# se-hwan/landing-controller

Hardware: AMD Instinct MI355X
Metric: landing NLPs solved/sec (SRBM, N=40, batch) (higher is better)
Workload: dtype f64

## Files before the change

landing-controller_amd/csrc/ipm_core.hpp:

```cpp
#pragma once
#include <hip/hip_runtime.h>
#include <math.h>

#include "../../include/landing_nlp.h"

namespace landing {

enum { RSUM = 0, RMAX = 1, RMIN = 2 };
__device__ __forceinline__ double red_op(double a, double b, int op) { return op == RSUM ? a + b : (op == RMAX ? fmax(a, b) : fmin(a, b)); }
template <int K>
__device__ __forceinline__ void block_reduce(double (&v)[K], const int (&op)[K], double* red) {
  const int tid = threadIdx.x, nwave = (blockDim.x + 63) >> 6;
  for (int i = 0; i < K; ++i) {
#pragma unroll
    for (int mask = 32; mask >= 1; mask >>= 1) v[i] = red_op(v[i], __shfl_xor(v[i], mask), op[i]);
  }
  if ((tid & 63) == 0) for (int i = 0; i < K; ++i) red[(tid >> 6) * K + i] = v[i];
  __syncthreads();
  for (int i = 0; i < K; ++i) {
    double r = red[i];
    for (int w = 1; w < nwave; ++w) r = red_op(r, red[w * K + i], op[i]);
    v[i] = r;
  }
  __syncthreads();
}
__device__ __forceinline__ double block_reduce1(double v, int op, double* red) {
  double a[1] = {v}; const int o[1] = {op};
  block_reduce<1>(a, o, red);
  return a[0];
}

__device__ __forceinline__ void top4_push(double (&t)[4], double v) {
#pragma unroll
  for (int i = 0; i < 4; ++i) { const double hi = fmax(t[i], v); v = fmin(t[i], v); t[i] = hi; }
}
__device__ __forceinline__ void block_top4(double (&t)[4], double* red) {
  const int tid = threadIdx.x, nwave = (blockDim.x + 63) >> 6;
#pragma unroll
  for (int mask = 32; mask >= 1; mask >>= 1) {
    double o[4];
#pragma unroll
    for (int i = 0; i < 4; ++i) o[i] = __shfl_xor(t[i], mask);
#pragma unroll
    for (int i = 0; i < 4; ++i) top4_push(t, o[i]);
  }
  if ((tid & 63) == 0) for (int i = 0; i < 4; ++i) red[(tid >> 6) * 4 + i] = t[i];
  __syncthreads();
  for (int i = 0; i < 4; ++i) t[i] = red[i];
  for (int w = 1; w < nwave; ++w) for (int i = 0; i < 4; ++i) top4_push(t, red[w * 4 + i]);
  __syncthreads();
}

typedef double f64x4 __attribute__((vector_size(32)));

#if defined(__HIP_DEVICE_COMPILE__)
typedef const double __attribute__((address_space(1)))* landing_gptr;
#else
typedef const double* landing_gptr;
#endif

struct ElStep { double dz, dw, dn, da; };
__device__ __forceinline__ ElStep el_step(double sd, double a, double n, double z, double w, double mu, double rho_pen, double ds) {
  ElStep e;
  const double D = a + z * n / w, rn = z + w - rho_pen;
  e.dz = (mu - a * z - z * (mu - n * w + n * rn) / w - sd * z * ds) / D;
  e.dw = -e.dz - rn;
  e.dn = (mu - n * w - n * e.dw) / w;
  e.da = sd * ds + e.dn;
  return e;
}

struct IpmCtl {
  double mu, delta_last, th_max, c_pr, c_co, c_cm, c_ys, c_zs, c_nz, e_pr, e_du, e_co;
  double tau, omt, a_pr, a_du, th0, ph0, dphi, alpha, s_corr, delta, ft;
  long long tp;
  int nfilt, it, status, need_reg_streak, nreset, last_reset_it, ncrawl, clip_k_cur, last_mu_it, cutstreak, wd_count, first_failed, force_step;
  int accepted, armijo_step, fact_ok, skipped_zero, attempt;
  int stag, full_prev;
  double e_prev;
  int flag, fresh, ls_done, need_corr, fallback;
  int feas, feas_used, lim;
  int fjam, fstat; double v1_ref;
  double c_rn, f_vmax, f_v1;
  int n_feas, stalled, polished, hard_lim, want_entry; double th_entry, f_theq;
  double fdc;
};
enum { ACT_GO = 0, ACT_STOP = 1, ACT_RESET = 2, ACT_FEAS = 3, ACT_BACK = 4 };

__host__ __device__ __forceinline__ void ipm_init(IpmCtl& K, const landing_solver_opts& o) {
  K = IpmCtl{};
  K.mu = o.mu_init; K.c_nz = 1.0; K.omt = -1.0; K.e_prev = 1e300;
  K.status = LANDING_MAX_ITER; K.clip_k_cur = o.clip_k; K.lim = o.max_iter; K.hard_lim = o.max_iter > 0 ? 3 * o.max_iter : 0;
  K.fdc = o.feas_delta_dec > 0.0 ? o.feas_delta_dec : o.delta_dec;
}

__host__ __device__ __forceinline__ void ipm_errors(IpmCtl& K, const landing_solver_opts& o, double du) {
  const double pr = K.c_pr, co = K.c_co;
  if (K.feas) du = fmax(du, K.c_rn);
  K.e_pr = pr; K.e_du = du; K.e_co = co;
  if (o.stag_relief > 0) {
    const double E = fmax(pr, du);
    K.stag = (!K.feas && K.mu <= o.tol / 10.0 * 1.0000001 && K.full_prev && E > 0.5 * K.e_prev) ? K.stag + 1 : 0;
    K.e_prev = E;
  }
}

__host__ __device__ __forceinline__ void ipm_enter_phase(IpmCtl& K, const landing_solver_opts& o) {
  const int it = K.it;
  K.feas = 1; K.n_feas++; K.feas_used = K.n_feas >= o.feas_max ? 1 : 0; K.status = LANDING_MAX_ITER; K.lim = it + o.max_iter; if (K.lim > K.hard_lim) K.lim = K.hard_lim; K.fstat = -1; K.fjam = 0; K.want_entry = 1; K.fdc = o.feas_delta_dec > 0.0 ? o.feas_delta_dec : o.delta_dec;
  K.mu = o.mu_init; K.nfilt = 0; K.th_max = 0.0; K.delta_last = 0.0; K.need_reg_streak = 0; K.cutstreak = 0; K.force_step = 0; K.wd_count = 0;
  K.it = it + 1;
}

__host__ __device__ __forceinline__ void ipm_leave_phase(IpmCtl& K, const landing_solver_opts& o) {
  const int it = K.it;
  K.feas = 0; K.lim = it + (o.max_iter > 1 ? o.max_iter : 1); if (K.lim > K.hard_lim) K.lim = K.hard_lim; K.status = LANDING_MAX_ITER;
  K.mu = (o.feas_ret_push > 0.0 && o.feas_ret_mu > 0.0) ? o.feas_ret_mu : o.mu_init; K.fjam = 0; K.nfilt = 0; K.delta_last = 0.0; K.need_reg_streak = 0; K.wd_count = 0; K.th_max = 0.0; K.nreset = 0; K.last_reset_it = it; K.ncrawl = 0;
  K.cutstreak = 0; K.force_step = 0;
  K.it = it + 1;
}

__host__ __device__ __forceinline__ void ipm_restart(IpmCtl& K, const landing_solver_opts& o, bool stalled, bool lost) {
  const int it = K.it, nreset = K.nreset;
  K.last_reset_it = it;
  if (stalled) K.ncrawl++;
  K.nreset = nreset + 1;
  K.fresh = (((o.fresh_restart & 2) && nreset + 1 == 2) || ((o.fresh_restart & 1) && nreset + 1 == 1 && !stalled && !lost)) ? 1 : 0;
  if (K.fresh) { if (K.clip_k_cur > 1) K.clip_k_cur = 2; K.th_max = 0.0; }
  K.mu = o.mu_init; K.nfilt = 0; K.delta_last = 0.0; K.need_reg_streak = 0; K.wd_count = 0;
  K.it = it + 1;
}

__host__ __device__ __forceinline__ int ipm_decide(IpmCtl& K, const landing_solver_opts& o, bool failed) {
  const double pr = K.e_pr, du = K.e_du, co = K.e_co, mu = K.mu;
  const int it = K.it, nreset = K.nreset;
  int act = ACT_GO;
  bool give_up = false;
  if (K.feas) {
    const bool conv = fmax(du, fmax(pr, co)) <= o.tol;
    if (!(du < 1e300) || !(pr < 1e300) || !(co < 1e300)) { K.status = LANDING_NUMERICAL; act = ACT_STOP; }
    else if (K.f_vmax <= 1e-9 && pr <= o.tol) act = ACT_BACK;
    else if (conv && K.f_v1 > o.feas_cert) { K.status = LANDING_INFEASIBLE; act = ACT_STOP; }
    else if (conv) act = ACT_BACK;
    else if (o.feas_back > 0.0 && !K.feas_used && K.f_v1 + K.f_theq <= o.feas_back * K.th_entry) act = ACT_BACK;
    else if (o.feas_stat > 0) {
      const double v1 = K.f_v1;
      if (K.fstat < 0 || !(fabs(v1 - K.v1_ref) <= 0.05 * K.v1_ref)) { K.v1_ref = v1; K.fstat = 0; } else K.fstat++;
      if (K.fstat >= o.feas_stat && mu <= 1e-4 && pr <= 1e-3) {
        if (v1 <= o.feas_cert) act = ACT_BACK;
        else if (o.feas_polish > 0.0 && !K.polished) {
          K.polished = 1; K.fstat = -1; K.delta_last = o.feas_polish / (o.feas_delta_dec > 0.0 ? o.feas_delta_dec : o.delta_dec); K.need_reg_streak = 2;
        }
        else if (o.feas_resume && !K.stalled) { K.stalled = 1; K.feas_used = 1; act = ACT_BACK; }
        else { K.status = LANDING_STALLED; act = ACT_STOP; }
      }
    }
    if (act == ACT_GO && it >= K.lim) act = ACT_STOP;
    if (act == ACT_BACK) ipm_leave_phase(K, o);
  }
  else if (failed) { K.status = LANDING_NUMERICAL; give_up = true; }
  else if (!(du < 1e300) || !(pr < 1e300) || !(co < 1e300)) { K.status = LANDING_NUMERICAL; give_up = true; }
  else if (fmax(du, fmax(pr, co)) <= o.tol) { K.status = LANDING_CONVERGED; act = ACT_STOP; }
  else if (it >= K.lim) give_up = true;
  else if (du > o.reset_du && nreset >= o.max_resets && o.max_resets > 0) { K.status = LANDING_NUMERICAL; give_up = true; }
  else if (o.feas_jam > 0 && K.fjam >= o.feas_jam && pr > 1e-3 && o.feas_phase) { give_up = true; if (K.feas_used) K.stalled = 1; }
  else {
    const bool jam = du > o.reset_du && nreset < o.max_resets;
    const bool stalled = o.restart_period > 0 && it - K.last_reset_it >= o.restart_period && mu >= o.mu_init && nreset < o.max_resets && K.ncrawl < ((o.fresh_restart & 4) ? 2 : 1);
    const bool overreg = o.reset_delta > 0.0 && K.delta_last > o.reset_delta && nreset < o.max_resets;
    const bool lost = (o.fresh_restart & 8) && o.restart_period > 0 && mu < o.mu_init && pr > 1e-3 && nreset < o.max_resets &&
                      ((it - K.last_mu_it >= 2 * o.restart_period && it - K.last_reset_it >= o.restart_period) || K.wd_count >= 3);
    if (jam || stalled || overreg || lost) { act = ACT_RESET; ipm_restart(K, o, stalled, lost); }
  }
  if (give_up) {
    if (K.stalled) K.status = LANDING_STALLED;
    if (o.feas_phase && !K.feas_used && o.max_iter > 0 && it < K.hard_lim) {
      act = ACT_FEAS;
      ipm_enter_phase(K, o);
    } else act = ACT_STOP;
  }
  return act;
}

__host__ __device__ __forceinline__ bool ipm_barrier_update(IpmCtl& K, const landing_solver_opts& o, int nfree) {
  double sd = 1.0, sc = 1.0;
  if (o.barrier_smax > 0.0) {
    sd = fmax(o.barrier_smax, (K.c_ys + K.c_zs) / ((double)nfree + K.c_nz)) / o.barrier_smax;
    sc = fmax(o.barrier_smax, K.c_zs / K.c_nz) / o.barrier_smax;
  }
  const double mu = K.mu;
  if (fmax(K.e_du / sd, fmax(K.c_pr, K.c_cm / sc)) <= o.kappa_eps * mu && mu > o.tol / 10.0) {
    K.mu = fmax(o.tol / 10.0, fmin(o.kappa_mu * mu, pow(mu, o.theta_mu)));
    K.nfilt = 0; K.last_mu_it = K.it; K.wd_count = 0;
    return true;
  }
  K.tau = fmax(o.tau_min, 1.0 - mu);
  return false;
}

__host__ __device__ __forceinline__ double ipm_delta_dec(const IpmCtl& K, const landing_solver_opts& o) { return (K.feas && o.feas_delta_dec > 0.0) ? K.fdc : o.delta_dec; }

__host__ __device__ __forceinline__ void ipm_first_delta(IpmCtl& K, const landing_solver_opts& o, double dec, double floor) {
  const double dl = K.delta_last;
// ... 163 lines not shown
```

landing-controller_amd/csrc/solver_kernels.hip:

```cpp
#include <hip/hip_runtime.h>
#include <math.h>
#include <type_traits>

#include "../../include/landing_nlp.h"
#include "ipm_core.hpp"


namespace landing {

constexpr int NZ_JX = 0, NZ_JU = 157, NZ_JUN = 385, NZ_HX = 613, NZ_HU = 642, NZ_HUN = 802, NZ_TOT = 962;
constexpr int GS = 49;
constexpr int PS = 25;
constexpr int YS = 37;
constexpr int RIC_K = 0, RIC_KAP = 576, RIC_MT = 600, RIC_MV = 888, RIC_PX = 900, RIC_PV = 1188, RIC_STRIDE = 1200;
constexpr int RIC_FWD0 = 288, RIC_FWDN = 612;
constexpr int FILT_CAP = 64;
constexpr int SOLVER_NMAX = 96;
constexpr int SOLVER_THREADS = 256;
constexpr int RCG = 36;
constexpr int RUNC = 48;

constexpr int CX_SR = NZ_TOT + 48, CX_ONE = CX_SR + 208, CX_MONE = CX_ONE + 1, CX_ZERO = CX_ONE + 2, CX_LEN = CX_ONE + 3;
constexpr int ATAB_TB = 6, ATAB_LTMAX = 6;
constexpr int ASM_NSLOT = 512;
// ... 50 lines not shown

__device__ __forceinline__ MemberMem carve(const Layout& L, double* w) {
  MemberMem M;
  M.x = w; w += L.nx; M.xt = w; w += L.nx; M.dx = w; w += L.nx; M.gx = w; w += L.nx;
  M.g = w; w += L.ng; M.gt = w; w += L.ng; M.s = w; w += L.ng; M.ds = w; w += L.ng;
  M.zL = w; w += L.ng; M.zU = w; w += L.ng;
  M.y = w; w += L.ng; M.yn = w; w += L.ng;
  M.sig = w; w += L.ng; M.rho = w; w += L.ng;
  M.J = w; w += L.nnz_jac; M.H = w; w += L.nnz_hess; M.Hc = w; w += (size_t)L.N * RUNC; M.ric = w; w += (size_t)(L.N + 1) * RIC_STRIDE; M.cond = w; w += (size_t)L.N * RCG;
  M.en = w; w += L.ng; M.ep = w; w += L.ng; M.wn = w; w += L.ng; M.wp = w; w += L.ng;
  M.sig2 = w; w += L.ng; M.rho2 = w; w += L.ng;
  M.s2 = w; w += L.ng; M.zL2 = w; w += L.ng; M.zU2 = w; w += L.ng; M.y2 = w;
  return M;
}

__host__ __device__ __forceinline__ void mem_accept_swap(MemberMem& M) {
  double* t;
#define LANDING_SWAP(a, b) t = M.a; M.a = M.b; M.b = t
  LANDING_SWAP(s, s2); LANDING_SWAP(zL, zL2); LANDING_SWAP(zU, zU2); LANDING_SWAP(y, y2); LANDING_SWAP(sig, sig2); LANDING_SWAP(rho, rho2);
  LANDING_SWAP(g, gt); LANDING_SWAP(x, xt);
#undef LANDING_SWAP
}


constexpr int FWD_DXL_NMAX = 64;
constexpr int XCH = 112 * 4;
static_assert(2 * XCH >= 24 * YS, "A1 also holds Y (24 x YS)");
struct Lds {
  double G[48 * GS];
  double P[24 * PS];
  double A1[2 * XCH];
  double Ah[2 * 12 * YS];
  double gam[48], q[24], sig[24], w[48], dinv[24];
  double red[(SOLVER_THREADS / 64) * 9];
  double filt_th[FILT_CAP], filt_ph[FILT_CAP];
  double prof[32];
  int flag;
  int segb[SOLVER_NMAX * 8];
  double carry[ASM_NSLOT];
  double rcl[RCG];
  double jhl[CX_LEN];
  double dump[64];
  const unsigned long long* ctab; const unsigned long long* ccomb; int c_ml, c_mid, rc_on;
  double bnd_lb[36 + 2 * 104], bnd_ub[36 + 2 * 104];
  MemberMem M; Layout L; const double* p; int prof_on;
  IpmCtl ks;
  int clip_now, jamrun, action, fact_failed;
  int first_trial, fast;
  double nxt[6];
  unsigned long long atab_mid[ATAB_LTMAX * SOLVER_THREADS];
  unsigned long long acomb_mid[SOLVER_THREADS];
};
__shared__ Lds SH;
__device__ __forceinline__ MemberMem live_mem() {
  MemberMem M = SH.M;
#if defined(__HIP_DEVICE_COMPILE__)
  double** q = reinterpret_cast<double**>(&M);
#pragma unroll
  for (int i = 0; i < MEMBER_MEM_PTRS; ++i) {
    const unsigned long long a = (unsigned long long)q[i];
    const unsigned lo = (unsigned)__builtin_amdgcn_readfirstlane((int)(unsigned)a), hi = (unsigned)__builtin_amdgcn_readfirstlane((int)(unsigned)(a >> 32));
    q[i] = (double*)((unsigned long long)lo | ((unsigned long long)hi << 32));
  }
#endif
  return M;
}
static_assert(36 * FWD_DXL_NMAX + 12 <= 24 * PS + 2 * XCH + 2 * 12 * YS && offsetof(Lds, A1) == offsetof(Lds, P) + sizeof(double) * 24 * PS && offsetof(Lds, Ah) == offsetof(Lds, A1) + sizeof(double) * 2 * XCH,
              "dx (x layout, N <= FWD_DXL_NMAX) fits the adjacent arrays [P | A1 | A^] (forward_pass / row_products)");
static_assert(offsetof(Lds, atab_mid) <= 65528, "the assembly tables address G, A^, gamma, cx, the partial sums and the dump slots with 16-bit byte offsets");
__host__ __device__ inline unsigned long long aterm_pack(int pa, int pb, int pc, int d, bool keep, bool ah) {
  const unsigned lo = (unsigned)pa | ((unsigned)pb << 16);
  const unsigned hi = (unsigned)pc | (((unsigned)d | (keep ? 1u : 0u) | (ah ? 2u : 0u)) << 16);
  return (unsigned long long)lo | ((unsigned long long)hi << 32);
}
__host__ __device__ inline unsigned long long acomb_pack(int n, int s0, int d, bool ah) {
  return (unsigned long long)((unsigned)n | ((unsigned)s0 << 16)) | ((unsigned long long)((unsigned)d | (ah ? 2u : 0u)) << 32);
}

template <int KT, class FA, class FB>
__device__ __forceinline__ f64x4 mfma_tile(f64x4 c, FA fa, FB fb) {
  const int l = threadIdx.x & 63, ij = l & 15, kq = l >> 4;
#pragma unroll
  for (int kt = 0; kt < KT; ++kt) c = __builtin_amdgcn_mfma_f64_16x16x4f64(fa(ij, kt * 4 + kq), fb(kt * 4 + kq, ij), c, 0, 0, 0);
  return c;
}

__device__ __forceinline__ double fast_rcp(double d) {
  double i = __builtin_amdgcn_rcp(d);
  i = fma(i, fma(-d, i, 1.0), i);
  return fma(i, fma(-d, i, 1.0), i);
}

__device__ __forceinline__ double lane_bcast(double v, int src) {
  const int hi = __builtin_amdgcn_readlane(__double2hiint(v), src);
  const int lo = __builtin_amdgcn_readlane(__double2loint(v), src);
  return __hiloint2double(hi, lo);
}

template <int NU>
__device__ __noinline__ void gauss_jordan_wave(const double* G, const double* gam, double* Kl, double* kl, int* flag) {
  const int lane = threadIdx.x;
  double col[NU];
  const bool isUU = lane < NU, isUS = lane >= NU && lane < NU + 24, isG = lane == NU + 24;
  {
    const double* src = isG ? gam + 24 : G + 24 * GS + (isUU ? 24 + lane : (isUS ? lane - NU : 0));
    const int stride = isG ? 1 : GS;
#pragma unroll
    for (int i = 0; i < NU; ++i) col[i] = src[i * stride];
  }
  bool ok = true;
#pragma unroll 1
  for (int j = 0; j < NU; ++j) {
    const double d = lane_bcast(col[0], j);
    if (!(d > 0.0) || !(d < 1e300)) ok = false;
    double inv = __builtin_amdgcn_rcp(d);
    inv = fma(inv, fma(-d, inv, 1.0), inv);
    inv = fma(inv, fma(-d, inv, 1.0), inv);
    const double pj = col[0] * inv;
    double m[NU];
#pragma unroll
    for (int i = 1; i < NU; ++i) m[i] = lane_bcast(col[i], j);
    __builtin_amdgcn_sched_barrier(0);
#pragma unroll
    for (int i = 1; i < NU; ++i) col[i - 1] = fma(-m[i], pj, col[i]);
    col[NU - 1] = pj;
  }
  if (isUS) {
#pragma unroll
    for (int i = 0; i < NU; ++i) Kl[i * 24 + (lane - NU)] = col[i];
  }
  if (isG) {
#pragma unroll
    for (int i = 0; i < NU; ++i) kl[i] = col[i];
  }
  if (lane == 0) *flag = ok ? 1 : 0;
}

constexpr int ASM_SEG_LEN[7] = {NZ_JU - NZ_JX, NZ_JUN - NZ_JU, NZ_HX - NZ_JUN, NZ_HU - NZ_HX, NZ_HUN - NZ_HU, NZ_TOT - NZ_HUN, RUNC};
constexpr int ASM_SEG_POS[7] = {NZ_JX, NZ_JU, NZ_JUN, NZ_HX, NZ_HU, NZ_HUN, NZ_TOT};
static_assert(NZ_JUN - NZ_JU <= SOLVER_THREADS && 2 * 104 <= SOLVER_THREADS, "one load per thread and segment");
__device__ __forceinline__ int uni(int v) {
#if defined(__HIP_DEVICE_COMPILE__)
  return __builtin_amdgcn_readfirstlane(v);
#else
  return v;
#endif
}
template <class P>
__device__ __forceinline__ P uni_ptr(P q) {
  const unsigned long long a = (unsigned long long)q;
  return (P)((unsigned long long)(unsigned)uni((int)(unsigned)a) | ((unsigned long long)(unsigned)uni((int)(unsigned)(a >> 32)) << 32));
}
__device__ __forceinline__ double uni(double v) { return __hiloint2double(uni(__double2hiint(v)), uni(__double2loint(v))); }
struct SweepCtx {
  landing_gptr JH, SR, Gr, Cd;
  const unsigned long long* ctab; const unsigned long long* ccomb;
  int c_ml, c_mid, rc_on, ng;
};
__device__ __forceinline__ SweepCtx sweep_ctx() {
  const Lds& S = SH;
  SweepCtx X;
  X.JH = uni_ptr((landing_gptr)S.M.J); X.SR = uni_ptr((landing_gptr)S.M.sig); X.Gr = uni_ptr((landing_gptr)S.M.g); X.Cd = uni_ptr((landing_gptr)S.M.cond);
  X.ctab = uni_ptr(S.ctab); X.ccomb = uni_ptr(S.ccomb);
  X.c_ml = uni(S.c_ml); X.c_mid = uni(S.c_mid); X.rc_on = uni(S.rc_on); X.ng = uni(S.L.ng);
  return X;
}
struct AsmRegs { double jh[7], sr, g, rc; int tp; };
__device__ __forceinline__ void asm_issue(int k, const SweepCtx& X, AsmRegs& R) {
  const Lds& S = SH;
  const int tid = threadIdx.x, ng = X.ng;
  const int* sb = S.segb + k * 8;
  const int g0 = Layout::g_stage(k);
#pragma unroll
  for (int sgm = 0; sgm < 7; ++sgm) R.jh[sgm] = X.JH[uni(sb[sgm]) + (tid < ASM_SEG_LEN[sgm] ? tid : 0)];
  R.tp = uni(sb[7]);
  R.sr = X.SR[tid < 104 ? g0 + tid : (tid < 208 ? ng + g0 + tid - 104 : 0)];
  R.g = X.Gr[g0 + (tid < 12 ? tid : 0)];
  R.rc = 0.0;
  if (X.rc_on) R.rc = X.Cd[(size_t)k * RCG + (tid < RCG ? tid : 0)];
}
__device__ __forceinline__ void asm_copy(const AsmRegs& R) {
  Lds& S = SH;
  const int tid = threadIdx.x;
#pragma unroll
  for (int sgm = 0; sgm < 7; ++sgm) if (tid < ASM_SEG_LEN[sgm]) S.jhl[ASM_SEG_POS[sgm] + tid] = R.jh[sgm];
  if (tid < 208) S.jhl[CX_SR + tid] = R.sr;
}
__device__ __forceinline__ void asm_terms(const SweepCtx& X, int nb, const AsmRegs& R) {
  Lds& S = SH;
  const int tid = threadIdx.x, LT = X.c_ml, tp = R.tp;
  char* const lds0 = reinterpret_cast<char*>(&S);
  const unsigned ahoff = nb ? (unsigned)(12 * YS * sizeof(double)) : 0u;
  const bool mid = (tp == X.c_mid);
  const unsigned long long* gt = X.ctab + (size_t)tp * LT * SOLVER_THREADS;
  double acc = 0.0;
  for (int j0 = 0; j0 < LT; j0 += ATAB_TB) {
    unsigned long long t[ATAB_TB];
    if (mid) {
#pragma unroll
      for (int u = 0; u < ATAB_TB; ++u) t[u] = S.atab_mid[(j0 + u) * SOLVER_THREADS + tid];
    } else {
#pragma unroll
      for (int u = 0; u < ATAB_TB; ++u) t[u] = gt[(j0 + u) * SOLVER_THREADS + tid];
    }
    double a[ATAB_TB], b[ATAB_TB], c[ATAB_TB];
#pragma unroll
    for (int u = 0; u < ATAB_TB; ++u) {
      const unsigned lo = (unsigned)t[u], hi = (unsigned)(t[u] >> 32);
      a[u] = *reinterpret_cast<const double*>(lds0 + (lo & 0xffffu)); b[u] = *reinterpret_cast<const double*>(lds0 + (lo >> 16)); c[u] = *reinterpret_cast<const double*>(lds0 + (hi & 0xffffu));
    }
#pragma unroll
    for (int u = 0; u < ATAB_TB; ++u) {
      const unsigned dd = (unsigned)(t[u] >> 48);
      acc += a[u] * b[u] * c[u];
      *reinterpret_cast<double*>(lds0 + ((dd & 0xfff8u) + ((dd & 2u) ? ahoff : 0u))) = acc;
      acc = (dd & 1u) ? acc : 0.0;
    }
  }
  if (tid < 12) { const int i = tid; S.Ah[nb * (12 * YS) + (i < 6 ? i : (i < 9 ? i + 3 : i - 3)) * YS + (YS - 1)] = -R.g; }
  if (tid < RCG) S.rcl[tid] = R.rc;
}
__device__ __forceinline__ void asm_combine(const SweepCtx& X, int nb, const AsmRegs& R) {
  Lds& S = SH;
  const int tid = threadIdx.x, tp = R.tp;
  const unsigned long long code = tp == X.c_mid ? S.acomb_mid[tid] : X.ccomb[tp * SOLVER_THREADS + tid];
  const unsigned lo = (unsigned)code, dd = (unsigned)(code >> 32);
  const int n = (int)(lo & 7u);
  if (n > 0) {
    char* const lds0 = reinterpret_cast<char*>(&S);
    const double* sl = reinterpret_cast<const double*>(lds0 + (lo >> 16));
    double tot = 0.0;
    for (int i = 0; i < n; ++i) tot += sl[i];
    *reinterpret_cast<double*>(lds0 + ((dd & 0xfff8u) + ((dd & 2u) ? (nb ? (unsigned)(12 * YS * sizeof(double)) : 0u) : 0u))) = tot;
  }
}

#if defined(__HIP_DEVICE_COMPILE__)
typedef double __attribute__((address_space(1)))* landing_gptr_w;
#else
typedef double* landing_gptr_w;
#endif
__device__ __forceinline__ landing_gptr_w uniform_record(double* rec) { return uni_ptr((landing_gptr_w)rec); }

constexpr int G_GAMMA = GS - 1, P_PV = PS - 1, AH_B = YS - 1;
static_assert(G_GAMMA == 48 && P_PV == 24 && AH_B == 36, "spare columns of G / P / A^ hold gamma / p / b");

template <int NU>
struct StageLanes {
  int ct, lj, lk, c;
  bool isg, live, ym, pm, wr;
  bool am[3];
  int gb, cd384, cm;
  int yb, pa1, pb, p2, fb, ab[3];
  int xw, xw0, xcp, xcr;
  unsigned iK, iM, iP, rs;
  int sw, pw;
};
template <int NU>
__device__ __forceinline__ StageLanes<NU> stage_lanes() {
  constexpr int NR = NU + 24, D = (int)sizeof(double);
  constexpr int oG = (int)offsetof(Lds, G), oP = (int)offsetof(Lds, P), oAh = (int)offsetof(Lds, Ah), oA1 = (int)offsetof(Lds, A1);
  StageLanes<NU> Z;
  const int tid = threadIdx.x, l = tid & 63;
  Z.ct = uni(tid >> 6); Z.lj = l & 15; Z.lk = l >> 4;
  const int ct = Z.ct, lj = Z.lj, lk = Z.lk, c = 16 * ct + lj;
  Z.c = c;
  Z.isg = (c == NR); Z.live = (c <= NR);
  const bool isg = Z.isg, live = Z.live;
  const int cl = c < NR ? c : NR;
  const int cp = NU == 24 ? cl : (cl < NU ? cl : cl + (24 - NU));
  Z.ym = live && (c < 12 || c >= NU);
  int ycol = c < NU ? c + 24 : c - NU;
  ycol = Z.ym ? (isg ? AH_B : ycol) : 0;
  Z.pm = live && c >= 12 && (c < NU || isg);
  const int pcol = Z.pm ? (isg ? P_PV : c) : 0;
  Z.gb = oG + (cp + lk * GS) * D; Z.cd384 = (cp - lk) * ((GS - 1) * D); Z.cm = c - lk;
  Z.yb = oAh + (lk * YS + ycol) * D;
  Z.pa1 = oP + (lj * PS + lk) * D;
  Z.pb = oP + (lk * PS + pcol) * D;
#pragma unroll
  for (int rt = 0; rt < 3; ++rt) {
    const int rho = 16 * rt + lj;
    const int a = rho < NU ? 24 + rho : (rho < NR ? rho - NU : 36);
    Z.am[rt] = a < 36;
    Z.ab[rt] = oAh + (lk * YS + (Z.am[rt] ? a : 0)) * D;
  }
  Z.p2 = oP + ((12 + (lj < 12 ? lj : 11)) * PS + lk) * D;
  Z.fb = oAh + ((lj < 12 ? lj : 11) * YS + 24 + lk) * D;
  Z.xw = oA1 + (c * 4 + lk) * D; Z.xw0 = oA1 + (c * 4) * D; Z.xcp = oA1 + (64 * 4 + lk * 4 + lj) * D; Z.xcr = oA1 + (64 * 4 + lj * 4 + lk) * D;
  Z.wr = c >= NU && c <= NR;
  const unsigned sj = (unsigned)(c - NU), ulk = (unsigned)lk, rs = isg ? 1u : 24u;
  Z.rs = rs * D;
  Z.iK = ((isg ? (unsigned)RIC_KAP : (unsigned)RIC_K + sj) + ulk * rs) * D; Z.iM = ((isg ? (unsigned)RIC_MV : (unsigned)RIC_MT + sj) + ulk * rs) * D;
  Z.iP = ((isg ? (unsigned)RIC_PV : (unsigned)RIC_PX + sj) + ulk * rs) * D;
  const int scol = isg ? AH_B : (int)sj, pcw = isg ? P_PV : (int)sj;
  Z.sw = oAh + (lk * YS + scol) * D; Z.pw = oP + (lk * PS + pcw) * D;
  return Z;
}
__device__ __forceinline__ double lds_get(int boff) { return *reinterpret_cast<const double*>(reinterpret_cast<const char*>(&SH) + boff); }
__device__ __forceinline__ void lds_put(int boff, double v) { *reinterpret_cast<double*>(reinterpret_cast<char*>(&SH) + boff) = v; }

constexpr unsigned PIVOT_KEY_MAX = 0x7e37e43cu - 0x00100000u;
template <int STEP, int NU>
__device__ __forceinline__ unsigned pivot_block_step(f64x4 (&T)[3], const StageLanes<NU>& Z) {
  constexpr int OFF = 4 * STEP, D = (int)sizeof(double);
  static_assert((OFF >> 4) == ((OFF + 3) >> 4), "a pivot block lies inside one row tile");
  constexpr int RTB = OFF >> 4, R0 = (OFF & 15) >> 2;
  constexpr int WSZ = 64 * 4;
  static_assert(WSZ + 48 * 4 <= XCH, "exchange buffer");
  constexpr int XB = (STEP & 1) * XCH * D;
  constexpr int CB = (int)offsetof(Lds, A1) + XB + WSZ * D;
  const bool inblk = (unsigned)(Z.lj - (OFF & 15)) < 4u;
  lds_put(Z.xw + XB, T[RTB][R0]);
  if (Z.ct == RTB && inblk) {
#pragma unroll
    for (int rt = 0; rt < 3; ++rt)
#pragma unroll
      for (int r = 0; r < 4; ++r) lds_put(Z.xcp + XB + ((16 * rt + 4 * r) * 4 - (OFF & 15)) * D, T[rt][r]);
  }
  __syncthreads();
  double a[4][4];
#pragma unroll
  for (int i = 0; i < 4; ++i)
#pragma unroll
    for (int j = 0; j <= i; ++j) a[i][j] = lds_get(CB + ((OFF + i) * 4 + j) * D);
  double w[4];
#pragma unroll
  for (int i = 0; i < 4; ++i) w[i] = lds_get(Z.xw0 + XB + i * D);
  double am[3];
#pragma unroll
  for (int rt = 0; rt < 3; ++rt) { const double cv = lds_get(Z.xcr + XB + 16 * rt * 4 * D); am[rt] = (rt == RTB && inblk) ? 0.0 : cv; }
  auto recip = [](double d) { double i = __builtin_amdgcn_rcp(d); i = fma(i, fma(-d, i, 1.0), i); return fma(i, fma(-d, i, 1.0), i); };
  const double a00 = a[0][0], a10 = a[1][0], a11 = a[1][1], a20 = a[2][0], a21 = a[2][1], a22 = a[2][2], a30 = a[3][0], a31 = a[3][1], a32 = a[3][2], a33 = a[3][3];
  const double detA = fma(a00, a11, -a10 * a10), iA = recip(detA);
  const double e00 = fma(a20, a11, -a21 * a10) * iA, e01 = fma(a21, a00, -a20 * a10) * iA, e10 = fma(a30, a11, -a31 * a10) * iA, e11 = fma(a31, a00, -a30 * a10) * iA;
  const double s00 = fma(-e01, a21, fma(-e00, a20, a22)), s10 = fma(-e11, a21, fma(-e10, a20, a32)), s11 = fma(-e11, a31, fma(-e10, a30, a33));
  const double detS = fma(s00, s11, -s10 * s10), iS = recip(detS);
  unsigned hm = 0u;
  { const double piv[4] = {a00, detA, s00, detS};
#pragma unroll
    for (int j = 0; j < 4; ++j) { const unsigned h = (unsigned)__double2hiint(piv[j]) - 0x00100000u; hm = h > hm ? h : hm; } }
  const int lk = Z.lk;
  auto solve = [&](const double (&wv)[4]) {
    const double t2 = fma(-e01, wv[1], fma(-e00, wv[0], wv[2])), t3 = fma(-e11, wv[1], fma(-e10, wv[0], wv[3]));
    const double r2 = fma(s11, t2, -s10 * t3) * iS, r3 = fma(s00, t3, -s10 * t2) * iS;
    const double q0 = fma(a11, wv[0], -a10 * wv[1]) * iA, q1 = fma(a00, wv[1], -a10 * wv[0]) * iA;
    const double r0 = fma(-e10, r3, fma(-e00, r2, q0)), r1 = fma(-e11, r3, fma(-e01, r2, q1));
    return lk == 0 ? r0 : (lk == 1 ? r1 : (lk == 2 ? r2 : r3));
  };
  const double R = solve(w);
  if (16 * Z.ct + 16 > OFF) {
#pragma unroll
    for (int rt = 0; rt < 3; ++rt) T[rt] = __builtin_amdgcn_mfma_f64_16x16x4f64(am[rt], -R, T[rt], 0, 0, 0);
    T[RTB][R0] = R;
  }
  return hm;
}

__device__ __forceinline__ void rec_put(landing_gptr_w rec, unsigned boff, double v) {
#if defined(__HIP_DEVICE_COMPILE__)
  typedef char __attribute__((address_space(1)))* gchar_w;
  *reinterpret_cast<landing_gptr_w>(reinterpret_cast<gchar_w>(rec) + boff) = v;
#else
  *reinterpret_cast<double*>(reinterpret_cast<char*>(rec) + boff) = v;
#endif
}
template <int NU>
__device__ __forceinline__ bool stage_eliminate(const StageLanes<NU>& Z, const SweepCtx& X, landing_gptr_w rec, double delta, int k) {
  constexpr int NR = NU + 24, D = (int)sizeof(double);
  const int lk = Z.lk;
  const bool isg = Z.isg, live = Z.live, ym = Z.ym, pm = Z.pm;
  const int cb = k & 1;
  const int ah = cb * (12 * YS * D);
  f64x4 T[3];
  {
#pragma unroll
    for (int rt = 0; rt < 3; ++rt)
#pragma unroll
      for (int r = 0; r < 4; ++r) {
        const int rb = 16 * rt + 4 * r;
        if (rb < NR) {
          const int rp = NU == 24 ? rb : (rb < NU ? rb : rb + (24 - NU));
          const int m384 = rp * ((GS - 1) * D) < Z.cd384 ? rp * ((GS - 1) * D) : Z.cd384;
          const double v = lds_get(Z.gb + rp * D + m384) + (Z.cm == rb ? delta : 0.0);
          T[rt][r] = live ? v : 0.0;
        } else T[rt][r] = 0.0;
      }
    if (X.rc_on) {
      Lds& S = SH;
#pragma unroll
      for (int rt = 0; rt < 3; ++rt)
#pragma unroll
        for (int r = 0; r < 4; ++r) {
          const int rb = 16 * rt + 4 * r;
          if (rb < NR) {
            const int ab = rb < NU ? 24 + rb : rb - NU;
            static_assert(RCG % 4 == 0 && NU % 4 == 0, "a group of four rows lies on one side of every border");
            const double g = ab < RCG ? S.rcl[ab + lk] : 0.0;
            T[rt][r] += isg ? g : 0.0;
          }
        }
    }
  }
  {
    double be[3];
    {
      const int yb = Z.yb + ah;
#pragma unroll
      for (int kt = 0; kt < 3; ++kt) { const double v = lds_get(yb + 4 * kt * YS * D); be[kt] = ym ? v : 0.0; }
    }
    double pa1[3], add1[3];
#pragma unroll
    for (int kt = 0; kt < 3; ++kt) pa1[kt] = lds_get(Z.pa1 + 4 * kt * D);
#pragma unroll
    for (int r = 0; r < 3; ++r) { const double v = lds_get(Z.pb + 4 * r * PS * D); add1[r] = pm ? v : 0.0; }
    double av[3][3];
#pragma unroll
    for (int rt = 0; rt < 3; ++rt) {
      const int ab = Z.ab[rt] + ah;
#pragma unroll
      for (int kt = 0; kt < 3; ++kt) { const double v = lds_get(ab + 4 * kt * YS * D); av[rt][kt] = Z.am[rt] ? v : 0.0; }
    }
    double pa2[3], add2[3];
    if (NU == 24) {
#pragma unroll
      for (int kt = 0; kt < 3; ++kt) pa2[kt] = lds_get(Z.p2 + 4 * kt * D);
#pragma unroll
      for (int r = 0; r < 3; ++r) { const double v = lds_get(Z.pb + (12 + 4 * r) * PS * D); add2[r] = pm ? v : 0.0; }
    }
    f64x4 Y1 = {0.0, 0.0, 0.0, 0.0};
#pragma unroll
    for (int kt = 0; kt < 3; ++kt) Y1 = __builtin_amdgcn_mfma_f64_16x16x4f64(pa1[kt], be[kt], Y1, 0, 0, 0);
#pragma unroll
    for (int r = 0; r < 3; ++r) Y1[r] += add1[r];
#pragma unroll
    for (int rt = 0; rt < 3; ++rt)
#pragma unroll
      for (int kt = 0; kt < 3; ++kt) T[rt] = __builtin_amdgcn_mfma_f64_16x16x4f64(av[rt][kt], Y1[kt], T[rt], 0, 0, 0);
    if (NU == 24) {
      f64x4 Y2 = {0.0, 0.0, 0.0, 0.0};
#pragma unroll
      for (int kt = 0; kt < 3; ++kt) Y2 = __builtin_amdgcn_mfma_f64_16x16x4f64(pa2[kt], be[kt], Y2, 0, 0, 0);
#pragma unroll
      for (int r = 0; r < 3; ++r) Y2[r] += add2[r];
      T[0][3] += Y2[0]; T[1][0] += Y2[1]; T[1][1] += Y2[2];
    }
  }
  static_assert(NU == 12 || NU == 24, "3 or 6 block steps per stage");
  constexpr int SC = NU == 24 ? 3 : 1;
  AsmRegs nxt;
  const bool more = k > 0;
#define ASM_HOOK(step) do { if constexpr (SC == (step)) { if (more) asm_copy(nxt); } if constexpr (SC + 1 == (step)) { if (more) asm_terms(X, cb ^ 1, nxt); } if constexpr (SC + 2 == (step)) { if (more) asm_combine(X, cb ^ 1, nxt); } } while (0)
  unsigned key = pivot_block_step<0>(T, Z), kq;
#define KEY_MAX(e) do { kq = (e); key = kq > key ? kq : key; } while (0)
  if (more) asm_issue(k - 1, X, nxt);
  ASM_HOOK(1);
  KEY_MAX(pivot_block_step<1>(T, Z));
  ASM_HOOK(2);
  KEY_MAX(pivot_block_step<2>(T, Z));
  ASM_HOOK(3);
  if constexpr (NU == 24) {
    KEY_MAX(pivot_block_step<3>(T, Z));
    ASM_HOOK(4);
    KEY_MAX(pivot_block_step<4>(T, Z));
    ASM_HOOK(5);
    KEY_MAX(pivot_block_step<5>(T, Z));
  }
#undef KEY_MAX
#undef ASM_HOOK
  if (!((unsigned)uni((int)key) < PIVOT_KEY_MAX)) return false;
  f64x4 Mq = {0.0, 0.0, 0.0, 0.0};
  {
    const int fb = Z.fb + ah;
#pragma unroll
    for (int kt = 0; kt < 3; ++kt) Mq = __builtin_amdgcn_mfma_f64_16x16x4f64(lds_get(fb + 4 * kt * D), T[0][kt], Mq, 0, 0, 0);
  }
  if (Z.wr) {
    const int sw = Z.sw + ah;
#pragma unroll
    for (int r = 0; r < 3; ++r) rec_put(rec, Z.iM + (unsigned)(4 * r) * Z.rs, lds_get(sw + 4 * r * YS * D) - Mq[r]);
#pragma unroll
    for (int rt = 0; rt < 3; ++rt)
#pragma unroll
      for (int r = 0; r < 4; ++r) {
        const int rb = 16 * rt + 4 * r;
        const double v = T[rt][r];
        if (rb < NU) rec_put(rec, Z.iK + (unsigned)rb * Z.rs, v);
        else if (rb < NR) {
          lds_put(Z.pw + (rb - NU) * PS * D, v);
          if (rb - NU < 12) rec_put(rec, Z.iP + (unsigned)(rb - NU) * Z.rs, v);
        }
      }
  }
  return true;
}

__device__ __noinline__ bool last_stage_eliminate(double* rec_, double delta_, int k_) {
  const StageLanes<12> Z = stage_lanes<12>();
  const SweepCtx X = sweep_ctx();
  return stage_eliminate<12>(Z, X, uniform_record(rec_), uni(delta_), uni(k_));
}

template <bool TIMED>
__device__ __forceinline__ bool stage_loop(const StageLanes<24>& Z, const SweepCtx& X, landing_gptr_w rec, double delta, int k, int& n_try) {
  bool ok = true;
  for (; k >= 0 && ok; --k, rec -= RIC_STRIDE) {
    long long tb_ = 0;
    if (TIMED) tb_ = (long long)wall_clock64();
    ok = stage_eliminate<24>(Z, X, rec, delta, k);
    __syncthreads();
    ++n_try;
    if (TIMED) { const long long n_ = (long long)wall_clock64(); if (threadIdx.x == 0) SH.prof[PH_B_ELIM] += (double)(n_ - tb_); }
  }
  return ok;
}

__device__ __noinline__ bool riccati_backward(double delta) {
  Lds& S = SH;
  const Layout& L = S.L;
  const MemberMem& M = S.M;
  const double* p = S.p;
  const int N = L.N, lane = threadIdx.x, NT = blockDim.x;
  (void)p; (void)N; (void)lane; (void)NT;
  bool ok = true;
  int n_try = 0;
  for (int e = lane; e < 24 * PS; e += NT) S.P[e] = 0.0;
  __syncthreads();
  if (lane < 12) {
    const int i = lane;
    const int ra = i < 6 ? 12 + i : 24 + (i - 6), rb = i < 6 ? 18 + i : 30 + (i - 6);
    const double qn2 = S.ks.feas ? 0.0 : 2.0 * p[L.o_QN + i];
    S.P[i * PS + i] = qn2 + M.sig[ra] + M.sig[rb] + delta;
    S.P[i * PS + P_PV] = qn2 * (M.x[12 * N + i] - p[12 * N + i]) + M.rho[ra] + M.rho[rb];
    double* rec = M.ric + (size_t)N * RIC_STRIDE;
    for (int j = 0; j < 24; ++j) rec[RIC_PX + i * 24 + j] = (j == i) ? S.P[i * PS + i] : 0.0;
    rec[RIC_PV + i] = S.P[i * PS + P_PV];
  }
  for (int e = lane; e < 48 * GS; e += NT) S.G[e] = 0.0;
  for (int e = lane; e < 2 * 12 * YS; e += NT) S.Ah[e] = 0.0;
  __syncthreads();
  const SweepCtx X = sweep_ctx();
  const bool timed = uni(S.prof_on) != 0;
  {
    AsmRegs first;
    asm_issue(N - 1, X, first);
    asm_copy(first);
    __syncthreads();
    asm_terms(X, (N - 1) & 1, first);
    __syncthreads();
    asm_combine(X, (N - 1) & 1, first);
  }
  __syncthreads();
  {
    long long tb_ = timed ? (long long)wall_clock64() : 0;
    ok = uni(last_stage_eliminate(M.ric + (size_t)(N - 1) * RIC_STRIDE, delta, N - 1) ? 1 : 0) != 0;
    __syncthreads();
    ++n_try;
    if (timed) { const long long n_ = (long long)wall_clock64(); if (lane == 0) S.prof[PH_B_ELIM] += (double)(n_ - tb_); }
  }
  if (ok && N > 1) {
    const StageLanes<24> Z = stage_lanes<24>();
    const int Nu = uni(N);
    const landing_gptr_w rec = uniform_record(M.ric) + (size_t)(Nu - 2) * RIC_STRIDE;
    const double du = uni(delta);
    ok = timed ? stage_loop<true>(Z, X, rec, du, Nu - 2, n_try) : stage_loop<false>(Z, X, rec, du, Nu - 2, n_try);
  }
  if (ok) {
    if (lane < 12) {
      const int i = lane;
      const double x0i = (i < 6) ? p[L.o_q_init + i] : p[L.o_qd_init + i - 6];
      S.sig[i] = x0i - M.x[i];
    }
    for (int e = lane; e < 144; e += NT) { const int i = e / 12, j = e % 12; S.G[(24 + i) * GS + 24 + j] = S.P[(12 + i) * PS + 12 + j]; }
    __syncthreads();
    if (lane < 12) {
      double v = S.P[(12 + lane) * PS + P_PV];
      for (int t = 0; t < 12; ++t) v += S.P[(12 + lane) * PS + t] * S.sig[t];
      S.gam[24 + lane] = v;
    }
    __syncthreads();
    if (lane < 64) gauss_jordan_wave<12>(S.G, S.gam, S.A1, S.A1 + 24 * 24, &S.flag);
    __syncthreads();
    ok = S.flag != 0;
    ++n_try;
    if (ok) {
      if (lane < 12) S.sig[12 + lane] = -S.A1[24 * 24 + lane];
      __syncthreads();
    }
  }
  if (lane == 0) { S.prof[PH_NSTAGE] += (double)n_try; S.prof[PH_NSTAGE_OK] += (double)(ok ? n_try : n_try - 1); }
  __syncthreads();
  return ok;
}

__device__ __noinline__ void forward_pass() {
  Lds& S = SH;
  const Layout& L = S.L;
  const MemberMem& M = S.M;
  const int N = L.N, tid = threadIdx.x, NT = blockDim.x;
  double* sg = S.G;
  double* buf = S.jhl;
  double* buf1 = S.A1;
  static_assert(24 * (SOLVER_NMAX + 1) <= 48 * GS && RIC_FWDN <= NZ_TOT + RUNC && RIC_FWDN <= XCH * 2, "forward scratch fits");
  auto slot = [&](int k) { return (k & 1) ? buf1 : buf; };
  auto fetch = [&](int k, double (&r)[3]) {
    landing_gptr rec = (landing_gptr)(M.ric + (size_t)(k < N ? k : N - 1) * RIC_STRIDE + RIC_FWD0);
#pragma unroll
    for (int j = 0; j < 3; ++j) { const int e = tid + j * 256; r[j] = rec[e < RIC_FWDN ? e : RIC_FWDN - 1]; }
  };
  auto stash = [&](int k, const double (&r)[3]) {
    double* b = slot(k);
#pragma unroll
    for (int j = 0; j < 3; ++j) { const int e = tid + j * 256; if (k < N && e < RIC_FWDN) b[e] = r[j]; }
  };
  if (tid < 24) sg[tid] = S.sig[tid];
  double r0[3], r1[3], r2[3], r3[3];
  fetch(0, r0); fetch(1, r1); fetch(2, r2); fetch(3, r3);
  stash(0, r0); fetch(4, r0);
  __syncthreads();
  auto stage = [&](int k, double (&rn)[3]) {
    if (k < N) {
      const double* b = slot(k);
      const bool lastk = (k == N - 1);
      if (tid < 192) {
        const int r = tid >> 3, j = tid & 7;
        const double* row = (r < 12) ? b + 312 + r * 24 : b + (r - 12) * 24;
        const double* sk = sg + 24 * k;
        double acc = row[3 * j] * sk[3 * j] + row[3 * j + 1] * sk[3 * j + 1] + row[3 * j + 2] * sk[3 * j + 2];
        acc += __shfl_xor(acc, 1); acc += __shfl_xor(acc, 2); acc += __shfl_xor(acc, 4);
        if (j == 0) sg[24 * (k + 1) + r] = (r < 12) ? b[600 + r] + acc : (lastk ? 0.0 : -(b[300 + (r - 12)] + acc));
      }
    }
    stash(k + 1, rn);
    fetch(k + 5, rn);
    __syncthreads();
  };
  for (int k0 = 0; k0 < N; k0 += 4) {
    stage(k0, r1); stage(k0 + 1, r2); stage(k0 + 2, r3); stage(k0 + 3, r0);
  }
  double* const dxl = S.P;
  const bool use_dxl = N <= FWD_DXL_NMAX;
  for (int e = tid; e < 24 * (N + 1); e += NT) {
    const int k = e / 24, i = e % 24;
    if (i < 12) { M.dx[L.x_X(k) + i] = sg[e]; if (use_dxl) dxl[L.x_X(k) + i] = sg[e]; }
    else if (k < N) { M.dx[L.x_U(k) + (i - 12)] = sg[e]; if (use_dxl) dxl[L.x_U(k) + (i - 12)] = sg[e]; }
  }
  for (int e = tid; e < 24 * N; e += NT) {
    const int k = e / 24, h = e % 24, i = h % 12;
    const double* sk = sg + 24 * (h < 12 ? k : k + 1);
    if (h < 12) {
      landing_gptr rec = (landing_gptr)(M.ric + (size_t)k * RIC_STRIDE);
      double acc = rec[RIC_KAP + i];
#pragma unroll
      for (int t = 0; t < 24; ++t) acc += rec[RIC_K + i * 24 + t] * sk[t];
      M.dx[L.x_U(k) + 12 + i] = -acc;
      if (use_dxl) dxl[L.x_U(k) + 12 + i] = -acc;
    } else {
      landing_gptr recn = (landing_gptr)(M.ric + (size_t)(k + 1) * RIC_STRIDE);
      double acc = recn[RIC_PV + i];
#pragma unroll
      for (int t = 0; t < 24; ++t) acc += recn[RIC_PX + i * 24 + t] * sk[t];
      const int q = i < 6 ? i : (i < 9 ? i + 3 : i - 3);
      M.yn[L.g_stage(k) + q] = -acc;
    }
  }
  if (tid < 12) {
    const int i = tid;
    const double v = sg[24 * N + i];
    const int ra = i < 6 ? 12 + i : 24 + (i - 6), rb = i < 6 ? 18 + i : 30 + (i - 6);
    M.ds[ra] = v + (M.g[ra] - M.s[ra]);
    M.ds[rb] = v + (M.g[rb] - M.s[rb]);
  }
  __syncthreads();
}

__device__ __noinline__ void row_products(const unsigned long long* __restrict__ rterm, int rlen) {
  Lds& S = SH;
  const MemberMem& M = S.M;
  const int tid = threadIdx.x, NT = blockDim.x;
  const double* __restrict__ Jn = M.J; const double* __restrict__ dxv = M.dx;
  const double* dxl = S.P; const bool use_dxl = S.L.N <= FWD_DXL_NMAX;
  double* __restrict__ dsv = M.ds;
  double acc = 0.0;
  constexpr int BW = 8;
  unsigned long long tn[BW];
#pragma unroll
  for (int u = 0; u < BW; ++u) tn[u] = (u < rlen) ? rterm[(size_t)u * NT + tid] : 0ull;
  for (int j0 = 0; j0 < rlen; j0 += BW) {
    unsigned long long t[BW];
#pragma unroll
    for (int u = 0; u < BW; ++u) t[u] = tn[u];
#pragma unroll
    for (int u = 0; u < BW; ++u) { const int j = j0 + BW + u; tn[u] = (j < rlen) ? rterm[(size_t)j * NT + tid] : 0ull; }
    double a[BW], b[BW];
#pragma unroll
    for (int u = 0; u < BW; ++u) {
      const int ij = (int)(t[u] & 0xffffu), ix = (int)((t[u] >> 16) & 0xffffu);
      a[u] = Jn[ij]; b[u] = use_dxl ? dxl[ix] : dxv[ix];
    }
#pragma unroll
    for (int u = 0; u < BW; ++u) {
      const bool valid = (t[u] >> 49) & 1ull, closes = (t[u] >> 48) & 1ull;
      acc += valid ? a[u] * b[u] : 0.0;
      if (closes) { dsv[(int)((t[u] >> 32) & 0xffffu)] = acc; acc = 0.0; }
    }
  }
  __syncthreads();
}

__device__ __noinline__ void rc_init_hc() {
  const Layout& L = SH.L; const double* p = SH.p;
  for (int e = threadIdx.x; e < L.N * RUNC; e += blockDim.x) {
    const int k = e / RUNC, j = e % RUNC, a = j % 3;
    const double dt2 = 2.0 * p[L.o_dt + k];
    double v;
    if (j < 12) v = dt2 * (rc_QX(L, p, j) + (j < 3 ? 4.0 * rc_Qc(L, p, j) : 0.0));
    else if (j < 24) v = -dt2 * rc_Qc(L, p, a);
    else if (j < 36) v = dt2 * rc_Qc(L, p, a);
    else v = dt2 * rc_Qf(L, p, a);
    SH.M.Hc[e] = v;
  }
}
__device__ __noinline__ void rc_add_grad() {
  const Layout& L = SH.L; const MemberMem& M = SH.M;
  for (int k = threadIdx.x; k < L.N; k += blockDim.x) { double* gU = M.gx + L.x_U(k); (void)run_cost_stage(L, M.x, SH.p, k, M.gx + L.x_X(k), gU, gU + 12); }
}
__device__ __noinline__ void rc_add_gamma() {
  const Layout& L = SH.L; const MemberMem& M = SH.M;
  for (int k = threadIdx.x; k < L.N; k += blockDim.x) {
    double gr[36];
#pragma unroll
    for (int a = 0; a < 36; ++a) gr[a] = 0.0;
    (void)run_cost_stage(L, M.x, SH.p, k, gr, gr + 12, gr + 24);
    double* gm = M.cond + (size_t)k * RCG;
#pragma unroll
    for (int a = 0; a < 36; ++a) gm[a] = gr[a];
  }
}
__device__ __noinline__ void rc_f_dphi(double& f0, double& dphi) {
  const Layout& L = SH.L; const MemberMem& M = SH.M;
  for (int k0 = 0; k0 < L.N; k0 += blockDim.x) {
    const int k = k0 + threadIdx.x;
    if (k >= L.N) continue;
    double gr[36];
#pragma unroll
    for (int a = 0; a < 36; ++a) gr[a] = 0.0;
    f0 += run_cost_stage(L, M.x, SH.p, k, gr, gr + 12, gr + 24);
    const double* dX = M.dx + L.x_X(k); const double* dU = M.dx + L.x_U(k);
#pragma unroll
    for (int a = 0; a < 12; ++a) dphi += gr[a] * dX[a] + gr[12 + a] * dU[a] + gr[24 + a] * dU[12 + a];
  }
}
__device__ __noinline__ double rc_f(const double* x) {
  const Layout& L = SH.L;
  double f = 0.0;
  for (int k0 = 0; k0 < L.N; k0 += blockDim.x) { const int k = k0 + threadIdx.x; if (k < L.N) f += run_cost_stage(L, x, SH.p, k, nullptr, nullptr, nullptr); }
  return f;
}

constexpr int SOLVER_MIN_WAVES = 2;
__global__ void landing_mpc_shift_kernel(Layout L, int B, const double* __restrict__ x_prev, const double* __restrict__ state,
                                         double* __restrict__ p, double* __restrict__ x0) {
  const size_t idx = (size_t)blockIdx.x * blockDim.x + threadIdx.x;
  if (idx >= (size_t)B * L.nx) return;
  const int m = (int)(idx / L.nx), i = (int)(idx % L.nx), N = L.N, nX = 12 * (N + 1);
  const double* xp = x_prev + (size_t)m * L.nx;
  double v;
  if (i < 12) v = state[(size_t)m * 12 + i];
  else if (i < nX) { const int k = i / 12, r = i % 12; v = xp[12 * (k < N ? k + 1 : N) + r]; }
  else { const int j = i - nX, k = j / 24, r = j % 24; v = xp[nX + 24 * (k < N - 1 ? k + 1 : N - 1) + r]; }
  x0[idx] = v;
  if (i < 6) p[(size_t)m * L.np + L.o_q_init + i] = v;
  else if (i < 12) p[(size_t)m * L.np + L.o_qd_init + (i - 6)] = v;
}

constexpr int ORDER_THREADS = 256;
__global__ void __launch_bounds__(ORDER_THREADS) landing_order_kernel(Layout L, int B, const double* __restrict__ p, int* __restrict__ order) {
  __shared__ double keys[ORDER_THREADS];
  const int tid = threadIdx.x, m = blockIdx.x * ORDER_THREADS + tid;
  const int off = L.o_q_init + 2;
  double key = m < B ? p[(size_t)m * L.np + off] : 0.0;
  if (!(key == key)) key = -INFINITY;
  int rank = 0;
// ... 595 lines not shown
```

Baseline: 22430.

## Prefetch assembly table words early and use DPP lane sums in forward pass

Assembly term and combine code words are now loaded during asm_copy and carried in registers, so asm_terms and asm_combine no longer issue their own global or LDS loads. The table walk becomes a single batch, guarded by a static_assert that the table length equals the batch size. The forward pass hoists per-thread row, bias and fetch offsets out of the stage loop. Its 8-lane reduction uses DPP moves in place of shuffles. The cost is higher register pressure from holding seven 64-bit words per thread across pipeline steps.

```diff
diff --git a/landing-controller_amd/csrc/ipm_core.hpp b/landing-controller_amd/csrc/ipm_core.hpp
--- a/landing-controller_amd/csrc/ipm_core.hpp
+++ b/landing-controller_amd/csrc/ipm_core.hpp
@@ -49,6 +49,25 @@
   for (int i = 0; i < 4; ++i) t[i] = red[i];
   for (int w = 1; w < nwave; ++w) for (int i = 0; i < 4; ++i) top4_push(t, red[w * 4 + i]);
   __syncthreads();
+}
+
+#if defined(__HIP_DEVICE_COMPILE__)
+template <int CTRL>
+__device__ __forceinline__ double dpp_move(double v) {
+  const int lo = __builtin_amdgcn_update_dpp(__double2loint(v), __double2loint(v), CTRL, 0xf, 0xf, false);
+  const int hi = __builtin_amdgcn_update_dpp(__double2hiint(v), __double2hiint(v), CTRL, 0xf, 0xf, false);
+  return __hiloint2double(hi, lo);
+}
+enum { DPP_QUAD_XOR1 = 0xb1, DPP_QUAD_XOR2 = 0x4e, DPP_ROW_SHL4 = 0x104 };
+#endif
+__device__ __forceinline__ double lane_sum8_head(double v) {
+#if defined(__HIP_DEVICE_COMPILE__)
+  v += dpp_move<DPP_QUAD_XOR1>(v); v += dpp_move<DPP_QUAD_XOR2>(v);
+  return v + dpp_move<DPP_ROW_SHL4>(v);
+#else
+  v += __shfl_xor(v, 1); v += __shfl_xor(v, 2);
+  return v + __shfl_xor(v, 4);
+#endif
 }
 
 typedef double f64x4 __attribute__((vector_size(32)));
diff --git a/landing-controller_amd/csrc/solver_kernels.hip b/landing-controller_amd/csrc/solver_kernels.hip
--- a/landing-controller_amd/csrc/solver_kernels.hip
+++ b/landing-controller_amd/csrc/solver_kernels.hip
@@ -226,20 +226,26 @@
   return (P)((unsigned long long)(unsigned)uni((int)(unsigned)a) | ((unsigned long long)(unsigned)uni((int)(unsigned)(a >> 32)) << 32));
 }
 __device__ __forceinline__ double uni(double v) { return __hiloint2double(uni(__double2hiint(v)), uni(__double2loint(v))); }
+#if defined(__HIP_DEVICE_COMPILE__)
+typedef const unsigned long long __attribute__((address_space(1)))* landing_gptr_u;
+#else
+typedef const unsigned long long* landing_gptr_u;
+#endif
 struct SweepCtx {
   landing_gptr JH, SR, Gr, Cd;
-  const unsigned long long* ctab; const unsigned long long* ccomb;
+  landing_gptr_u ctab, ccomb;
   int c_ml, c_mid, rc_on, ng;
 };
 __device__ __forceinline__ SweepCtx sweep_ctx() {
   const Lds& S = SH;
   SweepCtx X;
   X.JH = uni_ptr((landing_gptr)S.M.J); X.SR = uni_ptr((landing_gptr)S.M.sig); X.Gr = uni_ptr((landing_gptr)S.M.g); X.Cd = uni_ptr((landing_gptr)S.M.cond);
-  X.ctab = uni_ptr(S.ctab); X.ccomb = uni_ptr(S.ccomb);
+  X.ctab = uni_ptr((landing_gptr_u)S.ctab); X.ccomb = uni_ptr((landing_gptr_u)S.ccomb);
   X.c_ml = uni(S.c_ml); X.c_mid = uni(S.c_mid); X.rc_on = uni(S.rc_on); X.ng = uni(S.L.ng);
   return X;
 }
-struct AsmRegs { double jh[7], sr, g, rc; int tp; };
+static_assert(ATAB_LTMAX == ATAB_TB, "a thread's terms of a stage are ONE batch: its words travel in AsmRegs");
+struct AsmRegs { double jh[7], sr, g, rc; int tp; unsigned long long tw[ATAB_TB], cw; };
 __device__ __forceinline__ void asm_issue(int k, const SweepCtx& X, AsmRegs& R) {
   const Lds& S = SH;
   const int tid = threadIdx.x, ng = X.ng;
@@ -253,30 +259,32 @@
   R.rc = 0.0;
   if (X.rc_on) R.rc = X.Cd[(size_t)k * RCG + (tid < RCG ? tid : 0)];
 }
-__device__ __forceinline__ void asm_copy(const AsmRegs& R) {
+__device__ __forceinline__ void asm_copy(const SweepCtx& X, int nb, AsmRegs& R) {
   Lds& S = SH;
   const int tid = threadIdx.x;
 #pragma unroll
   for (int sgm = 0; sgm < 7; ++sgm) if (tid < ASM_SEG_LEN[sgm]) S.jhl[ASM_SEG_POS[sgm] + tid] = R.jh[sgm];
   if (tid < 208) S.jhl[CX_SR + tid] = R.sr;
-}
-__device__ __forceinline__ void asm_terms(const SweepCtx& X, int nb, const AsmRegs& R) {
+  if (tid < 12) { const int i = tid; S.Ah[nb * (12 * YS) + (i < 6 ? i : (i < 9 ? i + 3 : i - 3)) * YS + (YS - 1)] = -R.g; }
+  if (tid < RCG) S.rcl[tid] = R.rc;
+  if (R.tp == X.c_mid) {
+#pragma unroll
+    for (int u = 0; u < ATAB_TB; ++u) R.tw[u] = S.atab_mid[u * SOLVER_THREADS + tid];
+    R.cw = S.acomb_mid[tid];
+  } else {
+    const landing_gptr_u gt = X.ctab + (size_t)R.tp * X.c_ml * SOLVER_THREADS;
+#pragma unroll
+    for (int u = 0; u < ATAB_TB; ++u) R.tw[u] = gt[u * SOLVER_THREADS + tid];
+    R.cw = X.ccomb[R.tp * SOLVER_THREADS + tid];
+  }
+}
+__device__ __forceinline__ void asm_terms(int nb, const AsmRegs& R) {
   Lds& S = SH;
-  const int tid = threadIdx.x, LT = X.c_ml, tp = R.tp;
   char* const lds0 = reinterpret_cast<char*>(&S);
   const unsigned ahoff = nb ? (unsigned)(12 * YS * sizeof(double)) : 0u;
-  const bool mid = (tp == X.c_mid);
-  const unsigned long long* gt = X.ctab + (size_t)tp * LT * SOLVER_THREADS;
   double acc = 0.0;
-  for (int j0 = 0; j0 < LT; j0 += ATAB_TB) {
-    unsigned long long t[ATAB_TB];
-    if (mid) {
-#pragma unroll
-      for (int u = 0; u < ATAB_TB; ++u) t[u] = S.atab_mid[(j0 + u) * SOLVER_THREADS + tid];
-    } else {
-#pragma unroll
-      for (int u = 0; u < ATAB_TB; ++u) t[u] = gt[(j0 + u) * SOLVER_THREADS + tid];
-    }
+  {
+    const unsigned long long (&t)[ATAB_TB] = R.tw;
     double a[ATAB_TB], b[ATAB_TB], c[ATAB_TB];
 #pragma unroll
     for (int u = 0; u < ATAB_TB; ++u) {
@@ -291,13 +299,10 @@
       acc = (dd & 1u) ? acc : 0.0;
     }
   }
-  if (tid < 12) { const int i = tid; S.Ah[nb * (12 * YS) + (i < 6 ? i : (i < 9 ? i + 3 : i - 3)) * YS + (YS - 1)] = -R.g; }
-  if (tid < RCG) S.rcl[tid] = R.rc;
-}
-__device__ __forceinline__ void asm_combine(const SweepCtx& X, int nb, const AsmRegs& R) {
+}
+__device__ __forceinline__ void asm_combine(int nb, const AsmRegs& R) {
   Lds& S = SH;
-  const int tid = threadIdx.x, tp = R.tp;
-  const unsigned long long code = tp == X.c_mid ? S.acomb_mid[tid] : X.ccomb[tp * SOLVER_THREADS + tid];
+  const unsigned long long code = R.cw;
   const unsigned lo = (unsigned)code, dd = (unsigned)(code >> 32);
   const int n = (int)(lo & 7u);
   if (n > 0) {
@@ -524,7 +529,7 @@
   constexpr int SC = NU == 24 ? 3 : 1;
   AsmRegs nxt;
   const bool more = k > 0;
-#define ASM_HOOK(step) do { if constexpr (SC == (step)) { if (more) asm_copy(nxt); } if constexpr (SC + 1 == (step)) { if (more) asm_terms(X, cb ^ 1, nxt); } if constexpr (SC + 2 == (step)) { if (more) asm_combine(X, cb ^ 1, nxt); } } while (0)
+#define ASM_HOOK(step) do { if constexpr (SC == (step)) { if (more) asm_copy(X, cb ^ 1, nxt); } if constexpr (SC + 1 == (step)) { if (more) asm_terms(cb ^ 1, nxt); } if constexpr (SC + 2 == (step)) { if (more) asm_combine(cb ^ 1, nxt); } } while (0)
   unsigned key = pivot_block_step<0>(T, Z), kq;
 #define KEY_MAX(e) do { kq = (e); key = kq > key ? kq : key; } while (0)
   if (more) asm_issue(k - 1, X, nxt);
@@ -618,11 +623,11 @@
   {
     AsmRegs first;
     asm_issue(N - 1, X, first);
-    asm_copy(first);
+    asm_copy(X, (N - 1) & 1, first);
     __syncthreads();
-    asm_terms(X, (N - 1) & 1, first);
+    asm_terms((N - 1) & 1, first);
     __syncthreads();
-    asm_combine(X, (N - 1) & 1, first);
+    asm_combine((N - 1) & 1, first);
   }
   __syncthreads();
   {
@@ -671,16 +676,20 @@
   Lds& S = SH;
   const Layout& L = S.L;
   const MemberMem& M = S.M;
-  const int N = L.N, tid = threadIdx.x, NT = blockDim.x;
+  const int N = uni(L.N), tid = threadIdx.x, NT = blockDim.x;
   double* sg = S.G;
   double* buf = S.jhl;
   double* buf1 = S.A1;
   static_assert(24 * (SOLVER_NMAX + 1) <= 48 * GS && RIC_FWDN <= NZ_TOT + RUNC && RIC_FWDN <= XCH * 2, "forward scratch fits");
   auto slot = [&](int k) { return (k & 1) ? buf1 : buf; };
+  const landing_gptr fwd0 = (landing_gptr)uniform_record(M.ric) + RIC_FWD0;
+  int fe[3];
+#pragma unroll
+  for (int j = 0; j < 3; ++j) { const int e = tid + j * 256; fe[j] = e < RIC_FWDN ? e : RIC_FWDN - 1; }
   auto fetch = [&](int k, double (&r)[3]) {
-    landing_gptr rec = (landing_gptr)(M.ric + (size_t)(k < N ? k : N - 1) * RIC_STRIDE + RIC_FWD0);
-#pragma unroll
-    for (int j = 0; j < 3; ++j) { const int e = tid + j * 256; r[j] = rec[e < RIC_FWDN ? e : RIC_FWDN - 1]; }
+    const landing_gptr rec = fwd0 + (size_t)(k < N ? k : N - 1) * RIC_STRIDE;
+#pragma unroll
+    for (int j = 0; j < 3; ++j) r[j] = rec[fe[j]];
   };
   auto stash = [&](int k, const double (&r)[3]) {
     double* b = slot(k);
@@ -692,17 +701,25 @@
   fetch(0, r0); fetch(1, r1); fetch(2, r2); fetch(3, r3);
   stash(0, r0); fetch(4, r0);
   __syncthreads();
+  const int fr = tid >> 3, fj = tid & 7;
+  const bool frow = tid < 192, fstate = fr < 12, fhead = frow && fj == 0;
+  const int f_row = (fstate ? 312 + fr * 24 : (fr - 12) * 24) + 3 * fj;
+  const int f_bias = fstate ? 600 + fr : 300 + (fr - 12);
   auto stage = [&](int k, double (&rn)[3]) {
     if (k < N) {
       const double* b = slot(k);
       const bool lastk = (k == N - 1);
-      if (tid < 192) {
-        const int r = tid >> 3, j = tid & 7;
-        const double* row = (r < 12) ? b + 312 + r * 24 : b + (r - 12) * 24;
-        const double* sk = sg + 24 * k;
-        double acc = row[3 * j] * sk[3 * j] + row[3 * j + 1] * sk[3 * j + 1] + row[3 * j + 2] * sk[3 * j + 2];
-        acc += __shfl_xor(acc, 1); acc += __shfl_xor(acc, 2); acc += __shfl_xor(acc, 4);
-        if (j == 0) sg[24 * (k + 1) + r] = (r < 12) ? b[600 + r] + acc : (lastk ? 0.0 : -(b[300 + (r - 12)] + acc));
+      if (frow) {
+        const double* row = b + f_row;
+        const double* sk = sg + 24 * k + 3 * fj;
+        double bias = b[f_bias];
+        double prod = row[0] * sk[0] + row[1] * sk[1] + row[2] * sk[2];
+#if defined(__HIP_DEVICE_COMPILE__)
+        asm volatile("" : "+v"(bias), "+v"(prod));
+#endif
+        const double acc = lane_sum8_head(prod);
+        const double v = bias + acc;
+        if (fhead) sg[24 * (k + 1) + fr] = fstate ? v : (lastk ? 0.0 : -v);
       }
     }
     stash(k + 1, rn);
```

Result: faster. 23050 (median of 6 runs) (+2.7%).
